# Jaureguy760/HaploHyped-VarAwareML

Hardware: AMD Instinct MI355X
Metric: variants/sec encode+compress, 3M-variant x 2.5k-sample VCF (higher is better)
Workload: dtype u8

## Files before the change

haplohyped_varawareml_amd/csrc/lz4bits.hip:

```cpp
#include "common.h"

#define BP_N 4096
#ifndef BP_MAXONES
#define BP_MAXONES 636
#endif
#ifndef BP_STAGE
#define BP_STAGE 576
#endif
#ifndef BP_WAVES
#define BP_WAVES 7
#endif
#define BP_QCAP 100
#ifndef BP_MAXONES_EXC
#define BP_MAXONES_EXC 540
#endif
#ifndef BP_STAGE_EXC
#define BP_STAGE_EXC 448
#endif
template <bool EXC> struct BpCfg {
    static constexpr uint32_t MAXONES = EXC ? BP_MAXONES_EXC : BP_MAXONES;
    static constexpr uint32_t STAGE = EXC ? BP_STAGE_EXC : BP_STAGE;
    static constexpr uint32_t PTRASH = MAXONES + 7;
};
#define BP_HLOG 6
#define BP_GAPCLIP 40
#define BP_MINM 6
#define BP_TMIN 4
#define BP_BACK 64
#define BP_STEPS 16
#define BP_PICK 3
#define BP_LAZY_MIN 3
#ifdef BP_MARKS
#define BP_MARK(name) asm volatile("; ==MARK " name)
#else
#define BP_MARK(name)
#endif
#ifndef BP_SKIP
#define BP_SKIP 0
#endif
#define BP_MFLIMIT (BP_N - 12)
#define BP_MATCHLIMIT (BP_N - 5)

template <bool CHAIN, bool EXC> struct BpLds {
    uint32_t bm[132];
    uint32_t xm[EXC ? 132 : 1];
    uint32_t cls[EXC ? 24 : 1];
    uint32_t tab[1 << BP_HLOG];
    uint8_t flag[72];
    uint16_t wpre[64];
    uint16_t P[BpCfg<EXC>::MAXONES + 8];
    uint16_t chain[CHAIN ? BpCfg<EXC>::MAXONES + 8 : 4];
    uint32_t gbw[(BpCfg<EXC>::MAXONES + 16) / 4];
    uint2 queue[BP_QCAP + 1];
    uint8_t stage[BpCfg<EXC>::STAGE + 8];
};

__device__ __forceinline__ uint2 bp_entry(uint32_t E, uint32_t msr, bool onM, bool onT, uint32_t rs, uint32_t re, uint32_t off)
{
    return make_uint2(E | ((msr & 0x1FFFu) << 13) | (onM ? 1u << 26 : 0u) | (onT ? 1u << 27 : 0u) | ((rs - E) << 28), re | (off << 13));
}

__device__ __forceinline__ uint32_t bp_row_shr(uint32_t x, int d)
{
    switch (d) {
    case 1: return (uint32_t)__builtin_amdgcn_update_dpp(0, (int)x, 0x111, 0xf, 0xf, false);
    case 2: return (uint32_t)__builtin_amdgcn_update_dpp(0, (int)x, 0x112, 0xf, 0xf, false);
    case 4: return (uint32_t)__builtin_amdgcn_update_dpp(0, (int)x, 0x114, 0xf, 0xf, false);
    default: return (uint32_t)__builtin_amdgcn_update_dpp(0, (int)x, 0x118, 0xf, 0xf, false);
    }
}

__device__ __forceinline__ uint32_t bp_scan_sum(uint32_t x, uint32_t lane)
{
    x += bp_row_shr(x, 1);
    x += bp_row_shr(x, 2);
    x += bp_row_shr(x, 4);
    x += bp_row_shr(x, 8);
    const uint32_t t0 = (uint32_t)__builtin_amdgcn_readlane((int)x, 15);
    const uint32_t t1 = (uint32_t)__builtin_amdgcn_readlane((int)x, 31) + t0;
    const uint32_t t2 = (uint32_t)__builtin_amdgcn_readlane((int)x, 47) + t1;
    const uint32_t row = lane >> 4;
    return x + (row == 0u ? 0u : (row == 1u ? t0 : (row == 2u ? t1 : t2)));
}

__device__ __forceinline__ uint32_t bp_max(uint32_t a, uint32_t b) { return a > b ? a : b; }

__device__ __forceinline__ uint32_t bp_scan_max(uint32_t x, uint32_t lane)
{
    x = bp_max(x, bp_row_shr(x, 1));
    x = bp_max(x, bp_row_shr(x, 2));
    x = bp_max(x, bp_row_shr(x, 4));
    x = bp_max(x, bp_row_shr(x, 8));
    const uint32_t t0 = (uint32_t)__builtin_amdgcn_readlane((int)x, 15);
    const uint32_t t1 = bp_max((uint32_t)__builtin_amdgcn_readlane((int)x, 31), t0);
    const uint32_t t2 = bp_max((uint32_t)__builtin_amdgcn_readlane((int)x, 47), t1);
    const uint32_t row = lane >> 4;
    return bp_max(x, row == 0u ? 0u : (row == 1u ? t0 : (row == 2u ? t1 : t2)));
}

__device__ __forceinline__ uint32_t bp_bits(const uint32_t *bm, uint32_t q)
{
    const uint32_t i = q >> 5;
    const uint32_t lo = bm[i], hi = bm[i + 1];
    return __builtin_amdgcn_alignbit(hi, lo, q & 31u);
}

__device__ __forceinline__ uint32_t bp_gap4(const uint32_t *gbw, uint32_t i)
{
    const uint32_t w = i >> 2;
    return __builtin_amdgcn_alignbit(gbw[w + 1u], gbw[w], (i & 3u) << 3);
}

__device__ __forceinline__ uint32_t bp_len_ext(uint32_t x) { return __umul24(x + 240u, 32897u) >> 23; }

template <bool EXC> __device__ __forceinline__ uint32_t bp_lit(uint32_t b, uint32_t x, uint32_t k)
{
    const uint32_t v = (b >> k) & 1u;
    return EXC ? (((x >> k) & 1u) ? 0xF7u : v) : v;
}

#ifndef BP_EMITSKIP
#define BP_EMITSKIP 0
#endif
template <bool EXC, bool TR, typename OUT>
__device__ __forceinline__ void bp_put_seq(const uint32_t *bm, const uint32_t *xm, OUT out, uint32_t tr, uint32_t at, uint32_t anchor,
                                           uint32_t start, uint32_t len, uint32_t off, bool on, uint32_t lane)
{
    const uint32_t ll = on ? start - anchor : 0u, ml = len - 4u;
    const uint32_t llx = on ? bp_len_ext(ll) : 0u, mlx = on ? bp_len_ext(ml) : 0u;
    if (BP_EMITSKIP == 3) return;
    const uint32_t lit = at + 1u + llx, o = lit + ll;
    const uint32_t tok = ((ll < 15u ? ll : 15u) << 4) | (ml < 15u ? ml : 15u);
    if (TR) {
        out[on ? at : tr] = (uint8_t)tok;
        out[on ? o : tr] = (uint8_t)(off & 0xFFu);
        out[on ? o + 1u : tr] = (uint8_t)(off >> 8);
        out[llx != 0u ? at + 1u : tr] = (uint8_t)(llx == 1u ? ll - 15u : 255u);
        out[mlx != 0u ? o + 2u : tr] = (uint8_t)(mlx == 1u ? ml - 15u : 255u);
    } else {
        if (on) {
            out[at] = (uint8_t)tok;
            out[o] = (uint8_t)(off & 0xFFu);
            out[o + 1u] = (uint8_t)(off >> 8);
        }
        if (llx != 0u) out[at + 1u] = (uint8_t)(llx == 1u ? ll - 15u : 255u);
        if (mlx != 0u) out[o + 2u] = (uint8_t)(mlx == 1u ? ml - 15u : 255u);
    }
    if (__builtin_expect(__builtin_amdgcn_ballot_w64(llx > 1u || mlx > 1u) != 0ull, 0)) {
        uint32_t r = ll - 15u - 255u;
#pragma clang loop unroll(disable) vectorize(disable) interleave(disable)
        for (uint32_t k = 1; k < llx; ++k) {
            out[at + 1u + k] = (uint8_t)(k + 1u == llx ? r : 255u);
            r -= 255u;
        }
        r = ml - 15u - 255u;
#pragma clang loop unroll(disable) vectorize(disable) interleave(disable)
        for (uint32_t k = 1; k < mlx; ++k) {
            out[o + 2u + k] = (uint8_t)(k + 1u == mlx ? r : 255u);
            r -= 255u;
        }
    }
    if (BP_EMITSKIP != 1 && __builtin_amdgcn_ballot_w64(ll != 0u) != 0ull) {
        const uint32_t b = bp_bits(bm, anchor), x = EXC ? bp_bits(xm, anchor) : 0u;
        const uint32_t nsm = ll <= 6u ? ll : 0u;
#pragma unroll
        for (uint32_t k = 0; k < 6u; ++k) {
            if (TR) out[k < nsm ? lit + k : tr] = (uint8_t)bp_lit<EXC>(b, x, k);
            else if (k < nsm) out[lit + k] = (uint8_t)bp_lit<EXC>(b, x, k);
        }
        unsigned long long big = BP_EMITSKIP == 2 ? 0ull : __builtin_amdgcn_ballot_w64(ll > 6u);
        while (big != 0ull) {
            const int l = __builtin_ctzll(big);
            big &= big - 1ull;
            const uint32_t n = (uint32_t)__builtin_amdgcn_readlane((int)ll, l);
            const uint32_t src = (uint32_t)__builtin_amdgcn_readlane((int)anchor, l);
            const uint32_t dst = (uint32_t)__builtin_amdgcn_readlane((int)lit, l);
            for (uint32_t k = lane; k < n; k += 64u) out[dst + k] = (uint8_t)bp_lit<EXC>(bp_bits(bm, src + k), EXC ? bp_bits(xm, src + k) : 0u, 0u);
        }
    }
}

__device__ __forceinline__ void bp_flush(const uint8_t *stage, uint8_t *__restrict__ dst, uint32_t n, uint32_t lane)
{
    struct __attribute__((packed)) PU32 {
        uint32_t v;
    };
    const uint32_t nd = n >> 2;
    for (uint32_t i = lane; i < nd; i += 64u) reinterpret_cast<PU32 *>(dst + 4u * i)->v = reinterpret_cast<const uint32_t *>(stage)[i];
    const uint32_t t = (nd << 2) + lane;
    if (t < n) dst[t] = stage[t];
}

#define BP_FENCE() asm volatile("" ::: "memory")
struct BpOut {
    uint32_t prev_end, gop, sop;
};

template <bool EXC, typename LDS>
__device__ __forceinline__ BpOut bp_emit_batch(LDS &S, const uint32_t *bm, uint8_t *__restrict__ out, uint32_t n, uint32_t qn, BpOut st, uint32_t lane)
{
    const uint32_t *xm = S.xm;
    uint32_t prev_end = st.prev_end, gop = st.gop, sop = st.sop;
    const bool have = lane < n;
    uint2 en = S.queue[lane];
    en.x = have ? en.x : 0u;
    en.y = have ? en.y : 0u;
    const uint32_t E = en.x & 0x1FFFu, msr = (en.x >> 13) & 0x1FFFu, rs = E + (en.x >> 28), re = en.y & 0x1FFFu, off = en.y >> 13;
    const bool onM = (en.x >> 26) & 1u;
    bool onT = (en.x >> 27) & 1u;
    {
        uint32_t nx = S.queue[lane + 1u].x;
        nx = lane + 1u < qn ? nx : 0u;
        const uint32_t nmsr = (nx >> 13) & 0x1FFFu;
        const bool nM = (nx >> 26) & 1u;
        uint32_t nbk = nM && nmsr <= re ? re - nmsr : 0u;
        const uint32_t zt = re - rs;
        nbk = nbk < zt ? nbk : zt;
        onT = onT && zt - nbk >= BP_TMIN;
    }
    const uint32_t F0 = onT ? re : E;
    uint32_t Fp = (uint32_t)__builtin_amdgcn_update_dpp(0, (int)F0, 0x138 , 0xf, 0xf, false);
    Fp = lane ? Fp : prev_end;
    const uint32_t F = (onM || onT) ? F0 : Fp;
    uint32_t pe = (uint32_t)__builtin_amdgcn_update_dpp(0, (int)F, 0x138 , 0xf, 0xf, false);
    pe = lane ? pe : prev_end;
    uint32_t ms = msr > pe ? msr : pe;
    ms = onM ? ms : 0u;
    const uint32_t llM = onM ? ms - pe : 0u, lenM = E - ms;
    const uint32_t pe2 = onM ? E : pe;
    const uint32_t llT = onT ? rs - pe2 : 0u, lenT = re - rs;
    const uint32_t szM = onM ? 3u + bp_len_ext(llM) + llM + bp_len_ext(lenM - 4u) : 0u;
    const uint32_t szT = onT ? 3u + bp_len_ext(llT) + llT + bp_len_ext(lenT - 4u) : 0u;
    const uint32_t sincl = bp_scan_sum(szM + szT, lane);
    const uint32_t total = (uint32_t)__builtin_amdgcn_readlane((int)sincl, 63);
    BP_MARK("sizes_done");
    if (__builtin_expect(sop + total > BpCfg<EXC>::STAGE, 0)) {
        bp_flush(S.stage, out + gop, sop, lane);
        gop += sop;
        sop = 0;
    }
    const uint32_t at = sincl - (szM + szT);
    if (__builtin_expect(total > BpCfg<EXC>::STAGE, 0)) {
        bp_put_seq<EXC, false>(bm, xm, out + gop, 0u, at, pe, ms, lenM, off, onM, lane);
        bp_put_seq<EXC, false>(bm, xm, out + gop, 0u, at + szM, pe2, rs, lenT, 1u, onT, lane);
        gop += total;
    } else {
        bp_put_seq<EXC, true>(bm, xm, S.stage + sop, BpCfg<EXC>::STAGE - sop, at, pe, ms, lenM, off, onM, lane);
        bp_put_seq<EXC, true>(bm, xm, S.stage + sop, BpCfg<EXC>::STAGE - sop, at + szM, pe2, rs, lenT, 1u, onT, lane);
        sop += total;
    }
    prev_end = (uint32_t)__builtin_amdgcn_readlane((int)F, (int)(n - 1u));
    return BpOut{prev_end, gop, sop};
}

template <int DEPTH, bool EXC, bool LAZY, typename LDS>
__device__ __forceinline__ void bp_code_plane(LDS &S, uint32_t wlo, uint32_t whi, uint32_t xlo, uint32_t xhi, bool nonbinary, uint32_t bid,
                                              uint32_t wave, uint32_t lane, uint8_t *__restrict__ scratch, uint64_t slot_bytes,
                                              uint32_t *__restrict__ csize, uint32_t *__restrict__ flags, uint32_t tag)
{
    constexpr bool CHAIN = DEPTH > 1;
    uint32_t sink = 0;
    uint32_t *bm = S.bm;
    uint16_t *P = S.P;
    uint16_t *wpre = S.wpre;
    uint8_t *flag = S.flag;
    const uint64_t sidx = (uint64_t)bid * 2u + wave;
    uint8_t *out = scratch + sidx * slot_bytes;

    const uint32_t cnt = (uint32_t)__popc(wlo) + (uint32_t)__popc(whi);
    const uint32_t incl = bp_scan_sum(cnt, lane);
    const uint32_t m = (uint32_t)__builtin_amdgcn_readlane((int)incl, 63);
    if (nonbinary || m > BpCfg<EXC>::MAXONES) {
        if (lane == 0 && flags && flags[0] != tag) flags[0] = tag;
        if (lane == 0) csize[sidx] = 0xFFFFFFFFu;
        return;
    }
    BP_MARK("scan_done");
    wpre[lane] = (uint16_t)(incl - cnt);
    BP_FENCE();
    {
        uint32_t lo = wlo, hi = whi, at = incl - cnt + 1u;
        P[lane == 0u ? 0u : BpCfg<EXC>::PTRASH] = 0;
        uint32_t base = 64u * lane + 1u;
        while (__builtin_amdgcn_ballot_w64(lo != 0u) != 0ull) {
            const bool on = lo != 0u;
            const uint32_t bpos = (uint32_t)__builtin_ctz(lo | 0x80000000u);
            if (EXC && on && ((xlo >> bpos) & 1u)) atomicOr(&S.cls[at >> 5], 1u << (at & 31u));
            P[on ? at : BpCfg<EXC>::PTRASH] = (uint16_t)(base + bpos);
            at += on ? 1u : 0u;
            lo &= lo - 1u;
        }
        base += 32u;
        while (__builtin_amdgcn_ballot_w64(hi != 0u) != 0ull) {
            const bool on = hi != 0u;
            const uint32_t bpos = (uint32_t)__builtin_ctz(hi | 0x80000000u);
            if (EXC && on && ((xhi >> bpos) & 1u)) atomicOr(&S.cls[at >> 5], 1u << (at & 31u));
            P[on ? at : BpCfg<EXC>::PTRASH] = (uint16_t)(base + bpos);
            at += on ? 1u : 0u;
            hi &= hi - 1u;
        }
        P[lane < 4u ? m + 1u + lane : BpCfg<EXC>::PTRASH] = (uint16_t)(BP_N + 1);
    }
    BP_FENCE();
    if (DEPTH > 0) {
        uint8_t *gb = reinterpret_cast<uint8_t *>(S.gbw);
        for (uint32_t i = lane; i < m + 8u; i += 64u) {
            const uint32_t i1 = i + 1u < BpCfg<EXC>::PTRASH ? i + 1u : BpCfg<EXC>::PTRASH;
            uint32_t g = (uint32_t)P[i1] - (uint32_t)P[i1 - 1u] - 1u;
            g = g < 255u ? g : 255u;
            gb[i] = (uint8_t)(i < m ? g : 255u);
        }
        BP_FENCE();
    }
#pragma unroll
    for (int k = 0; k < (1 << BP_HLOG) / 64; ++k) S.tab[64 * k + lane] = 0u;

    BP_MARK("plist_done");
    if (BP_SKIP >= 4) {
        if (lane == 0) csize[sidx] = P[m] & 1u;
        return;
    }
    uint32_t gop = 0, sop = 0, prev_end = 0, qn = 0;
    int cur = -1;
    for (int jw = -1; jw < (int)m; jw += 64) {
        BP_MARK("win_begin");
#ifdef BP_PROBE_SALU
#pragma unroll
        for (int pr = 0; pr < BP_PROBE_SALU; ++pr) asm volatile("s_mov_b32 s90, 0" ::: "s90");
#endif
#ifdef BP_PROBE_VALU
        {
            uint32_t pv;
#pragma unroll
            for (int pr = 0; pr < BP_PROBE_VALU; ++pr) asm volatile("v_mov_b32 %0, 0" : "=v"(pv));
        }
#endif
        const int j = jw + (int)lane;
        const bool valid = j < (int)m;
        const uint32_t jj = valid ? (uint32_t)(j + 1) : 0u;
        const uint32_t q1 = P[jj], qn1 = P[jj + 1u];
        const uint32_t qp1 = jj ? P[jj - 1u] : 0u;
        const int q = (int)q1 - 1;
        const bool can = DEPTH > 0 && valid && j >= 0 && q + 12 <= BP_N;
        uint32_t jc1 = 0;
        const uint32_t c5a = EXC ? (bp_bits(S.cls, jj) & 31u) : 0u;
        if (can) {
            const uint32_t g1 = qn1 - q1;
            const uint32_t idx = (g1 < BP_GAPCLIP ? g1 : BP_GAPCLIP) ^ ((EXC && (c5a & 1u)) ? 63u : 0u);
            jc1 = atomicExch(&S.tab[idx], (uint32_t)(j + 1));
            if (CHAIN) S.chain[jj] = (uint16_t)jc1;
        }
        BP_FENCE();
        BP_MARK("hash_done");
        const uint32_t gq = q1 - qp1 - 1u;
        uint32_t len = 0, nb = 0, c1 = 0;
        bool hv = false;
        uint32_t a_last = jj;
        uint32_t z_last = 0;
        bool clamped = false;
        if (DEPTH > 0) {
            const uint32_t a4 = bp_gap4(S.gbw, jj);
            const uint8_t *gbb = reinterpret_cast<const uint8_t *>(S.gbw);
            const uint32_t fa = jj ? (uint32_t)gbb[jj - 1u] : 0u;
            const uint32_t na4 = ~a4;
            const uint32_t stop4 = ((na4 - 0x01010101u) & ~na4 & 0x80808080u) | 0xFF000000u;
            int best = -1;
            uint32_t bjq = 0, bk = 0;
#pragma unroll 1
            for (int dpt = 0; dpt < DEPTH; ++dpt) {
                const bool have = can && jc1 != 0u;
                if (__builtin_amdgcn_ballot_w64(have) == 0ull) break;
                const uint32_t jq = have ? jc1 : 1u;
                const uint32_t b4 = bp_gap4(S.gbw, jq);
                const uint32_t fb = (uint32_t)gbb[jq - 1u];
                uint32_t nextc = 0;
                if (CHAIN) nextc = S.chain[jq];
                const uint32_t x = (a4 ^ b4) | stop4;
                uint32_t k = (uint32_t)__builtin_ctz(x) >> 3;
                bool same = true;
                if (EXC) {
                    const uint32_t xc = c5a ^ (bp_bits(S.cls, jq) & 31u);
                    same = (xc & 1u) == 0u;
                    const uint32_t tv = (uint32_t)__builtin_ctz((xc >> 1) | 8u);
                    k = k < tv ? k : tv;
                }
                const uint32_t below = (1u << (8u * k)) - 1u;
                const uint32_t sumg = __builtin_amdgcn_sad_u8(a4 & below, 0u, k + 1u);
                const uint32_t za = (a4 >> (8u * k)) & 0xFFu, zb = (b4 >> (8u * k)) & 0xFFu;
                uint32_t fz = fa < fb ? fa : fb;
                fz = fz < BP_BACK ? fz : BP_BACK;
                const int score = (int)(sumg + (za < zb ? za : zb) + fz);
                const bool up = have & same & (score > best);
                best = up ? score : best;
                bjq = up ? jq : bjq;
                bk = up ? k : bk;
                if (!CHAIN) break;
                jc1 = have ? nextc : 0u;
            }
            const bool got = best >= 0;
            if (__builtin_amdgcn_ballot_w64(got) != 0ull) {
                const uint32_t jq = got ? bjq : 1u;
                const uint32_t cc1 = P[jq], cp1 = P[jq - 1u];
                uint32_t a = jj + bk, b = jq + bk;
                uint32_t pa = P[a], pb = P[b];
                uint32_t clen = pa - q1, costR = 0, tailz = 0, zl = 0;
#pragma unroll
                for (uint32_t s = 0; s < BP_PICK; ++s) {
                    const uint32_t g = (a4 >> (8u * s)) & 0xFFu;
                    costR += s < bk ? 1u + (g >= BP_TMIN + 1u ? 4u : g) : 0u;
                }
                bool act = got;
                for (uint32_t s = bk;; ++s) {
                    if (__builtin_amdgcn_ballot_w64(act) == 0ull) break;
                    const uint32_t na = P[a + 1u], nbn = P[b + 1u];
                    const uint32_t ga = na - pa - 1u, gb = nbn - pb - 1u;
                    const bool cdiff = EXC && (((bp_bits(S.cls, a + 1u) ^ bp_bits(S.cls, b + 1u)) & 1u) != 0u);
                    const bool stop = (s < BP_PICK) | (ga != gb) | (ga >= 255u) | (a >= m) | (s >= BP_STEPS) | cdiff;
                    const uint32_t z = ga < gb ? ga : gb;
                    costR += act ? 1u + (ga >= BP_TMIN + 1u ? 4u : ga) : 0u;
                    clen += act ? 1u + (stop ? z : ga) : 0u;
                    tailz = (act & stop) ? ga - z : tailz;
                    zl = (act & stop) ? z : zl;
                    act = act & !stop;
                    a += act ? 1u : 0u;
                    b += act ? 1u : 0u;
                    pa = act ? na : pa;
                    pb = act ? nbn : pb;
                }
                {
                    const uint32_t gc = cc1 - cp1 - 1u;
                    uint32_t cnb = gq < gc ? gq : gc;
                    cnb = cnb < BP_BACK ? cnb : BP_BACK;
                    const uint32_t costH = 3u + (clen + cnb >= 19u ? 1u : 0u) - cnb + (tailz >= BP_TMIN ? 3u : tailz);
                    uint32_t end = (uint32_t)q + clen;
                    clamped = end > BP_MATCHLIMIT;
                    end = end < BP_MATCHLIMIT ? end : BP_MATCHLIMIT;
                    const int gain = (int)costR - (int)costH;
                    hv = got & (gain > 0) & ((int)end - q >= 4) & ((int)end - (q - (int)cnb) >= BP_MINM) & (q <= BP_MFLIMIT);
                    len = hv ? end - (uint32_t)q : 0u;
                    nb = hv ? cnb : 0u;
                    c1 = hv ? cc1 : 0u;
                    a_last = a;
                    z_last = zl;
                    clamped = clamped & hv;
                }
            }
        }
        BP_MARK("cand_done");
        if (LAZY) {
            const uint32_t E0 = hv ? (uint32_t)q + len : (uint32_t)(q + 1);
            const uint32_t hvN = (uint32_t)__builtin_amdgcn_update_dpp(0, (int)(hv ? 1u : 0u), 0x130 , 0xf, 0xf, false);
            const uint32_t EN = (uint32_t)__builtin_amdgcn_update_dpp(0, (int)E0, 0x130, 0xf, 0xf, false);
            const uint32_t nbN = (uint32_t)__builtin_amdgcn_update_dpp(0, (int)nb, 0x130, 0xf, 0xf, false);
            const int msN = (int)qn1 - 1 - (int)nbN;
            const int between = msN - (int)q1 > 0 ? msN - (int)q1 : 0;
            const bool Ln = hv & (hvN != 0u) & (lane < 63u) & (j + 1 < (int)m) & (qn1 <= E0) & ((int)EN - (int)E0 >= (int)(BP_LAZY_MIN + nb) + between);
            const unsigned long long lm = __builtin_amdgcn_ballot_w64(Ln);
            const unsigned long long rest = ~(lm >> lane);
            const uint32_t tlo = (uint32_t)__builtin_ctz((uint32_t)rest | 0x80000000u), thi = (uint32_t)__builtin_ctz((uint32_t)(rest >> 32) | 0x80000000u);
            const uint32_t t = (uint32_t)rest != 0u ? tlo : 32u + thi;
            const bool give = Ln && (t & 1u);
            hv = hv && !give;
            len = give ? 0u : len;
            nb = give ? 0u : nb;
            c1 = give ? 0u : c1;
            a_last = give ? jj : a_last;
            z_last = give ? 0u : z_last;
            clamped = clamped && !give;
        }
        const uint32_t E = hv ? (uint32_t)q + len : (uint32_t)(q + 1);
        uint32_t nxt = hv ? a_last : jj;
        if (__builtin_amdgcn_ballot_w64(clamped) != 0ull) {
            const uint32_t w = E >> 6, bb = E & 63u, wc = w < 63u ? w : 63u;
            const uint32_t lo = bm[2u * wc], hi = bm[2u * wc + 1u];
            const uint32_t mlo = bb >= 32u ? 0xFFFFFFFFu : ((1u << bb) - 1u);
            const uint32_t mhi = bb > 32u ? ((1u << (bb - 32u)) - 1u) : 0u;
            const uint32_t in_map = (uint32_t)wpre[wc] + (uint32_t)__popc(lo & mlo) + (uint32_t)__popc(hi & mhi);
            nxt = clamped ? (w >= 64u ? m : in_map) : nxt;
        }
        BP_MARK("nxt_done");
        bool sel = false;
        if (BP_SKIP >= 3) {
            sink += nxt + E;
            continue;
        }
        if (cur < jw + 64) {
            const uint32_t e0 = (uint32_t)(cur - jw);
            uint32_t jump = valid ? (nxt - (uint32_t)jw < 64u ? nxt - (uint32_t)jw : 64u) : 64u;
            const uint32_t p0 = jump;
            flag[lane] = lane == e0 ? 1u : 0u;
            flag[lane == 0u ? 64u : 69u] = 0u;
            BP_FENCE();
            bool reach = lane == e0;
#pragma unroll
            for (int r = 0; r < 6; ++r) {
                flag[reach ? jump : 68u] = 1u;
                BP_FENCE();
                reach = flag[lane] != 0u;
                const uint32_t j2 = (uint32_t)__builtin_amdgcn_ds_bpermute((int)((jump & 63u) << 2), (int)jump);
                jump = jump < 64u ? j2 : 64u;
            }
            sel = reach && valid;
            const unsigned long long ex = __builtin_amdgcn_ballot_w64(sel && p0 == 64u);
            if (ex != 0ull) cur = (int)__builtin_amdgcn_readlane((int)nxt, (int)(__ffsll((long long)ex) - 1));
        }
        BP_MARK("sel_done");
        if (BP_SKIP >= 2) {
            sink += sel ? nxt : 0u;
            continue;
        }
        const bool onM = sel && hv;
        uint32_t rs = E + ((!hv || z_last == 0u) ? 1u : 0u);
        if (__builtin_amdgcn_ballot_w64(clamped) != 0ull)
            rs = clamped ? E + ((bp_bits(bm, E - 1u) & 1u) ? 1u : 0u) : rs;
        uint32_t re = (uint32_t)P[(nxt < m ? nxt : m) + 1u] - 1u;
        re = re < BP_MATCHLIMIT ? re : BP_MATCHLIMIT;
        const bool onT = sel && (int)re - (int)rs >= BP_TMIN && rs <= BP_MFLIMIT;
        const bool want = onM || onT;
        const unsigned long long wm = __builtin_amdgcn_ballot_w64(want);
        const uint32_t nw = (uint32_t)__builtin_popcountll(wm);
        const bool last = jw + 64 >= (int)m;
        for (int phase = 0; phase < 2; ++phase) {
            if (phase == 1) {
                const uint32_t slot = qn + __builtin_amdgcn_mbcnt_hi((uint32_t)(wm >> 32), __builtin_amdgcn_mbcnt_lo((uint32_t)wm, 0u));
                S.queue[want ? slot : (uint32_t)BP_QCAP] = bp_entry(E, (uint32_t)(q - (int)nb), onM, onT, rs, re, q1 - c1);
                qn += nw;
                BP_MARK("queued");
            }
            while (phase == 0 ? qn + nw > BP_QCAP : (qn >= 65u || (last && qn != 0u))) {
                const uint32_t keep = phase == 1 && last ? 0u : 1u;
                const uint32_t nb_ = qn - keep < 64u ? qn - keep : 64u;
                BP_FENCE();
                const BpOut r = bp_emit_batch<EXC>(S, bm, out, nb_, qn, BpOut{prev_end, gop, sop}, lane);
                prev_end = r.prev_end, gop = r.gop, sop = r.sop;
                BP_FENCE();
                const bool mvp = lane + nb_ < qn;
                const uint2 mv = S.queue[mvp ? nb_ + lane : (uint32_t)BP_QCAP];
                BP_FENCE();
                S.queue[mvp ? lane : (uint32_t)BP_QCAP] = mv;
                qn -= nb_;
            }
        }
        BP_MARK("emit_done");
    }
    BP_MARK("loop_done");
    if (BP_SKIP >= 1) {
        if (lane == 0) csize[sidx] = (prev_end + sink) & 0xFFFu;
        return;
    }
    {
        const uint32_t ll = BP_N - prev_end, llx = bp_len_ext(ll);
        BP_FENCE();
        if (sop + 1u + llx + ll > BpCfg<EXC>::STAGE) {
            bp_flush(S.stage, out + gop, sop, lane);
            gop += sop;
            sop = 0;
        }
        const bool direct = 1u + llx + ll > BpCfg<EXC>::STAGE;
        auto tail = [&](auto dstp) {
            if (lane == 0) {
                dstp[0] = (uint8_t)((ll < 15u ? ll : 15u) << 4);
                uint32_t r = ll - 15u;
                for (uint32_t k = 0; k < llx; ++k) {
                    dstp[1u + k] = (uint8_t)(k + 1u == llx ? r : 255u);
                    r -= 255u;
                }
            }
            for (uint32_t k = lane; k < ll; k += 64u)
                dstp[1u + llx + k] = (uint8_t)bp_lit<EXC>(bp_bits(bm, prev_end + k), EXC ? bp_bits(S.xm, prev_end + k) : 0u, 0u);
        };
        if (direct) {
            tail(out + gop);
            gop += 1u + llx + ll;
        } else {
            tail(S.stage + sop);
            sop += 1u + llx + ll;
        }
    }
    uint32_t op = gop + sop;
    if (op >= BP_N) {
        for (uint32_t k = lane; k < BP_N; k += 64u) out[k] = (uint8_t)bp_lit<EXC>(bp_bits(bm, k), EXC ? bp_bits(S.xm, k) : 0u, 0u);
        op = BP_N;
    } else {
        BP_FENCE();
        bp_flush(S.stage, out + gop, sop, lane);
    }
    if (BP_SKIP) op = (op & 0xFFFu) + (sink & 1u);
#ifdef BP_PROBE_HANDOFF
    {
        asm volatile("s_waitcnt vmcnt(0)" ::: "memory");
        uint32_t old = 0;
        if (lane == 0) old = atomicAdd(reinterpret_cast<uint32_t *>(scratch + (sidx & ~255ull) * slot_bytes + slot_bytes - 8u), 1u);
        old = (uint32_t)__builtin_amdgcn_readfirstlane((int)old);
        op += old == 0xFFFFFFF0u ? 1u : 0u;
    }
#endif
    if (lane == 0) csize[sidx] = op;
}

template <int DEPTH, bool LAZY = false>
__global__ __launch_bounds__(128, BP_WAVES) void k_lz4_bitplanes(const uint8_t *__restrict__ src, PlanesGeom pg, uint32_t n_blocks,
                                                                  uint8_t *__restrict__ scratch, uint64_t slot_bytes, uint32_t *__restrict__ csize,
                                                                  uint32_t *__restrict__ flags, uint32_t tag)
{
    constexpr bool CHAIN = DEPTH > 1;
    __shared__ BpLds<CHAIN, false> lds[2];
    __shared__ uint32_t nonbin[2][2];
    const uint32_t wave = (uint32_t)__builtin_amdgcn_readfirstlane((int)(threadIdx.x >> 6)), lane = threadIdx.x & 63u;
    const uint32_t bid = blockIdx.x;
    for (int once = 0; once < 1; ++once) {
    const uint8_t *blk = src + (uint64_t)bid * 8192u;

    {
        typedef uint32_t u32x4 __attribute__((ext_vector_type(4)));
        const u32x4 *p = reinterpret_cast<const u32x4 *>(blk + 4096u * wave + 16u * lane);
        u32x4 v[4];
#pragma unroll
        for (int k = 0; k < 4; ++k) v[k] = __builtin_nontemporal_load(p + 64 * k);
        uint32_t orall = 0;
        uint8_t *bm0 = reinterpret_cast<uint8_t *>(lds[0].bm) + 256u * wave + lane;
        uint8_t *bm1 = reinterpret_cast<uint8_t *>(lds[1].bm) + 256u * wave + lane;
#pragma unroll
        for (int k = 0; k < 4; ++k) {
            const uint32_t d[4] = {v[k].x, v[k].y, v[k].z, v[k].w};
            uint32_t acc0 = 0, acc1 = 0;
#pragma unroll
            for (int i = 0; i < 4; ++i) {
                const uint32_t x = d[i];
                orall |= x;
                const uint32_t xm = x & 0x01010101u;
                const uint32_t y = xm | (xm >> 15);
                acc0 |= (y & 3u) << (2 * i);
                acc1 |= ((y >> 8) & 3u) << (2 * i);
            }
            bm0[64 * k] = (uint8_t)acc0;
            bm1[64 * k] = (uint8_t)acc1;
        }
        const uint32_t nb0 = orall & 0x00FE00FEu, nb1 = orall & 0xFE00FE00u;
        const unsigned long long b0 = __builtin_amdgcn_ballot_w64(nb0 != 0u), b1 = __builtin_amdgcn_ballot_w64(nb1 != 0u);
        if (lane == 0) {
            nonbin[wave][0] = b0 != 0ull;
            nonbin[wave][1] = b1 != 0ull;
        }
        if (lane < 4u) lds[wave].bm[128u + lane] = 0u;
    }
    __syncthreads();
    const uint32_t wlo = lds[wave].bm[2u * lane], whi = lds[wave].bm[2u * lane + 1u];
    const bool nonbinary = (nonbin[0][wave] | nonbin[1][wave]) != 0u;
    BP_MARK("A_done");
    if (BP_SKIP >= 5) {
        if (lane == 0) csize[(uint64_t)bid * 2u + wave] = lds[wave].bm[5] & 1u;
        return;
    }

    bp_code_plane<DEPTH, false, LAZY>(lds[wave], wlo, whi, 0u, 0u, nonbinary, bid, wave, lane, scratch, slot_bytes, csize, flags, tag);
    }
}

template <int DEPTH, bool LAZY>
__global__ __launch_bounds__(128, BP_WAVES) void k_lz4_bitplanes_uni(const uint8_t *__restrict__ src, PlanesGeom pg, uint32_t n_blocks,
                                                                      uint8_t *__restrict__ scratch, uint64_t slot_bytes,
                                                                      uint32_t *__restrict__ csize, uint32_t *__restrict__ flags, uint32_t tag)
{
    constexpr bool CHAIN = DEPTH > 1;
    union BpBoth {
        BpLds<CHAIN, false> p;
        BpLds<CHAIN, true> x;
    };
    __shared__ BpBoth lds[2];
    const uint32_t wave = (uint32_t)__builtin_amdgcn_readfirstlane((int)(threadIdx.x >> 6)), lane = threadIdx.x & 63u;
    const uint32_t bid = (blockIdx.x & ~63u) | ((blockIdx.x & 7u) << 3) | ((blockIdx.x >> 3) & 7u);
    if (bid >= n_blocks) return;
    typedef uint32_t u32x2 __attribute__((ext_vector_type(2)));
    uint64_t col;
    uint32_t row, bi;
    planes_block(pg, bid, &col, &row, &bi);
    const u32x2 *pl = reinterpret_cast<const u32x2 *>(src + planes_piece(pg, col, bi * 16u + (lane >> 2), wave, row)) + (lane & 3u);
    const u32x2 one = *pl, exc = *(pl + (uint64_t)pg.S_pad * 8ull);
    if (__builtin_amdgcn_ballot_w64((exc.x | exc.y) != 0u) == 0ull) {
        BpLds<CHAIN, false> &S = lds[wave].p;
        S.bm[2u * lane] = one.x;
        S.bm[2u * lane + 1u] = one.y;
        if (lane < 4u) S.bm[128u + lane] = 0u;
        bp_code_plane<DEPTH, false, LAZY>(S, one.x, one.y, 0u, 0u, false, bid, wave, lane, scratch, slot_bytes, csize, flags, tag);
    } else {
        BpLds<CHAIN, true> &S = lds[wave].x;
        const bool nonbinary = __builtin_amdgcn_ballot_w64(((exc.x & ~one.x) | (exc.y & ~one.y)) != 0u) != 0ull;
        S.bm[2u * lane] = one.x;
        S.bm[2u * lane + 1u] = one.y;
        if (lane < 4u) S.bm[128u + lane] = 0u;
        S.xm[2u * lane] = exc.x;
        S.xm[2u * lane + 1u] = exc.y;
        if (lane < 4u) S.xm[128u + lane] = 0u;
        if (lane < 24u) S.cls[lane] = 0u;
        bp_code_plane<DEPTH, true, LAZY>(S, one.x, one.y, exc.x, exc.y, nonbinary, bid, wave, lane, scratch, slot_bytes, csize, flags, tag);
    }
}

int launch_lz4_bitplanes(const uint8_t *d_src, bool planes, PlanesGeom pg, uint64_t n_blocks, uint8_t *d_scratch, size_t slot_bytes, uint32_t *d_csize,
                         int depth, uint32_t *d_flags, uint32_t tag, hipStream_t st)
{
    const bool lazy = (depth & 0x100) != 0;
    depth &= 0xFF;
    if (n_blocks == 0) return HHGT_OK;
    if (n_blocks > 0x7fffffffull) {
        hhgt_set_error("lz4: too many blocks");
        return HHGT_ERR_ARG;
    }
#define BP_LAUNCH(D, LZ)                                                                                                    \
    do {                                                                                                                    \
        if (planes)                                                                                                         \
            hipLaunchKernelGGL((k_lz4_bitplanes_uni<D, LZ>), dim3((uint32_t)((n_blocks + 63) / 64 * 64)), dim3(128), 0, st, d_src, pg, \
                               (uint32_t)n_blocks, d_scratch, (uint64_t)slot_bytes, d_csize, d_flags, tag);                 \
        else                                                                                                                \
            hipLaunchKernelGGL((k_lz4_bitplanes<D, LZ>), dim3((uint32_t)n_blocks), dim3(128), 0, st, d_src, pg, (uint32_t)n_blocks, \
                               d_scratch, (uint64_t)slot_bytes, d_csize, d_flags, tag);                                     \
    } while (0)
    if (lazy && depth == 2) BP_LAUNCH(2, true);
    else if (lazy) BP_LAUNCH(12, true);
    else if (depth <= 0) BP_LAUNCH(0, false);
    else if (depth == 1) BP_LAUNCH(1, false);
    else if (depth == 2) BP_LAUNCH(2, false);
    else if (depth <= 4) BP_LAUNCH(4, false);
    else if (depth <= 8) BP_LAUNCH(8, false);
    else if (depth <= 12) BP_LAUNCH(12, false);
    else BP_LAUNCH(16, false);
#undef BP_LAUNCH
    HIP_TRY(hipGetLastError());
    return HHGT_OK;
}
```

Measured before the change: 152.7 million.

## Fuse gap-byte computation into position-list scatter and interleave lo/hi loops

Writes the gap bytes while scattering set-bit positions, so the separate gap pass over P and its extra fence are gone. The previous position carried across lanes comes from a max scan and a DPP shift. The lo and hi word loops are merged into one ballot loop with separate write cursors, which shortens the serial loop to the larger of the two popcounts. The cost is extra register state, a cross-lane scan, and more LDS stores per iteration, and correctness of the gap bytes now depends on the new lane-boundary logic.

```diff
diff --git a/haplohyped_varawareml_amd/csrc/lz4bits.hip b/haplohyped_varawareml_amd/csrc/lz4bits.hip
--- a/haplohyped_varawareml_amd/csrc/lz4bits.hip
+++ b/haplohyped_varawareml_amd/csrc/lz4bits.hip
@@ -279,39 +279,51 @@
     wpre[lane] = (uint16_t)(incl - cnt);
     BP_FENCE();
     {
-        uint32_t lo = wlo, hi = whi, at = incl - cnt + 1u;
+        constexpr uint32_t GTRASH = BpCfg<EXC>::MAXONES + 8u;
+        uint8_t *gb = reinterpret_cast<uint8_t *>(S.gbw);
+        const uint32_t base = 64u * lane + 1u;
+        uint32_t lo = wlo, hi = whi, alo = incl - cnt + 1u, ahi = alo + (uint32_t)__popc(wlo);
+        uint32_t plo = 0, phi = 0;
+        if (DEPTH > 0) {
+            const uint32_t llo = base + 31u - (uint32_t)__builtin_clz(wlo | 1u), lhi = base + 63u - (uint32_t)__builtin_clz(whi | 1u);
+            const uint32_t last = whi != 0u ? lhi : (wlo != 0u ? llo : 0u);
+            const uint32_t before = (uint32_t)__builtin_amdgcn_update_dpp(0, (int)bp_scan_max(last, lane), 0x138 , 0xf, 0xf, false);
+            plo = lane ? before : 0u;
+            phi = wlo != 0u ? llo : plo;
+        }
         P[lane == 0u ? 0u : BpCfg<EXC>::PTRASH] = 0;
-        uint32_t base = 64u * lane + 1u;
-        while (__builtin_amdgcn_ballot_w64(lo != 0u) != 0ull) {
-            const bool on = lo != 0u;
-            const uint32_t bpos = (uint32_t)__builtin_ctz(lo | 0x80000000u);
-            if (EXC && on && ((xlo >> bpos) & 1u)) atomicOr(&S.cls[at >> 5], 1u << (at & 31u));
-            P[on ? at : BpCfg<EXC>::PTRASH] = (uint16_t)(base + bpos);
-            at += on ? 1u : 0u;
-            lo &= lo - 1u;
-        }
-        base += 32u;
-        while (__builtin_amdgcn_ballot_w64(hi != 0u) != 0ull) {
-            const bool on = hi != 0u;
-            const uint32_t bpos = (uint32_t)__builtin_ctz(hi | 0x80000000u);
-            if (EXC && on && ((xhi >> bpos) & 1u)) atomicOr(&S.cls[at >> 5], 1u << (at & 31u));
-            P[on ? at : BpCfg<EXC>::PTRASH] = (uint16_t)(base + bpos);
-            at += on ? 1u : 0u;
-            hi &= hi - 1u;
+        while (__builtin_amdgcn_ballot_w64((lo | hi) != 0u) != 0ull) {
+            {
+                const bool on = lo != 0u;
+                const uint32_t bpos = (uint32_t)__builtin_ctz(lo | 0x80000000u), p1 = base + bpos;
+                if (EXC && on && ((xlo >> bpos) & 1u)) atomicOr(&S.cls[alo >> 5], 1u << (alo & 31u));
+                P[on ? alo : BpCfg<EXC>::PTRASH] = (uint16_t)p1;
+                if (DEPTH > 0) {
+                    const uint32_t g = p1 - plo - 1u;
+                    gb[on ? alo - 1u : GTRASH] = (uint8_t)(g < 255u ? g : 255u);
+                    plo = p1;
+                }
+                alo += on ? 1u : 0u;
+                lo &= lo - 1u;
+            }
+            {
+                const bool on = hi != 0u;
+                const uint32_t bpos = (uint32_t)__builtin_ctz(hi | 0x80000000u), p1 = base + 32u + bpos;
+                if (EXC && on && ((xhi >> bpos) & 1u)) atomicOr(&S.cls[ahi >> 5], 1u << (ahi & 31u));
+                P[on ? ahi : BpCfg<EXC>::PTRASH] = (uint16_t)p1;
+                if (DEPTH > 0) {
+                    const uint32_t g = p1 - phi - 1u;
+                    gb[on ? ahi - 1u : GTRASH] = (uint8_t)(g < 255u ? g : 255u);
+                    phi = p1;
+                }
+                ahi += on ? 1u : 0u;
+                hi &= hi - 1u;
+            }
         }
         P[lane < 4u ? m + 1u + lane : BpCfg<EXC>::PTRASH] = (uint16_t)(BP_N + 1);
+        if (DEPTH > 0) gb[lane < 8u ? m + lane : GTRASH] = 255u;
     }
     BP_FENCE();
-    if (DEPTH > 0) {
-        uint8_t *gb = reinterpret_cast<uint8_t *>(S.gbw);
-        for (uint32_t i = lane; i < m + 8u; i += 64u) {
-            const uint32_t i1 = i + 1u < BpCfg<EXC>::PTRASH ? i + 1u : BpCfg<EXC>::PTRASH;
-            uint32_t g = (uint32_t)P[i1] - (uint32_t)P[i1 - 1u] - 1u;
-            g = g < 255u ? g : 255u;
-            gb[i] = (uint8_t)(i < m ? g : 255u);
-        }
-        BP_FENCE();
-    }
 #pragma unroll
     for (int k = 0; k < (1 << BP_HLOG) / 64; ++k) S.tab[64 * k + lane] = 0u;
 
```

Result: no change. 152.3 million (-0.3%).
